# eezkni/UEGAN

Hardware: AMD Instinct MI355X
Metric: train imgs/sec @512px bs=16 on 1/2/4/8 MI355X; infer ms/img (higher is better)
Workload: dtype bf16; 1 GPU; FiveK-shaped 512x512 batch=16/GPU, full G/D/VGG train step (trainer.py:77-119), conv_dim=32, seeded stand-in VGG19; global_batch=16, parallelism=dp1, pool_size=50, collective=none (1 rank), passes=batched (fused.py)

## Files before the change

### uegan_amd/csrc/conv_wide.hip

```cpp
#include "conv_core.h"

namespace uegan {

static __device__ __attribute__((aligned(128))) const unsigned int g_zero_page[512] = {0u};

typedef float f32x16 __attribute__((ext_vector_type(16)));

__device__ __forceinline__ f32x16 mfma32_bf16(u32x4 a, u32x4 b, f32x16 c) {
#ifdef UEGAN_HALF_FP16
  return __builtin_amdgcn_mfma_f32_32x32x16_f16(__builtin_bit_cast(bf16x8_t, a), __builtin_bit_cast(bf16x8_t, b), c, 0, 0, 0);
#else
  return __builtin_amdgcn_mfma_f32_32x32x16_bf16(__builtin_bit_cast(bf16x8_t, a), __builtin_bit_cast(bf16x8_t, b), c, 0, 0, 0);
#endif
}

#define UEGAN_SB() __builtin_amdgcn_sched_barrier(0)

template <int KS, int MODE, bool MASK, int ABL = 0>
__global__ void __launch_bounds__(256, 1) conv_wide_kernel(ConvArgs a) {
  constexpr int TH = 8, TW = 32, BN = 256, NWAVES = 4;
  constexpr int PH = TH + KS - 1, PW = TW + KS - 1;
  constexpr int NPG = (PH * PW + 7) / 8;
  constexpr int NI_P = (NPG + NWAVES - 1) / NWAVES;
  constexpr int PBUFB = NPG * 1024, WHALF = BN * 64, DUMPB = 4096;
  constexpr int NT = KS * KS, NHC = 2 * NT;
  constexpr bool DGRAD = MODE != 0;
  static_assert(NI_P <= NHC - 2, "the next chunk's patch pieces must be requested two half steps before the chunk ends");
  static_assert(2 * PBUFB + 4 * WHALF + DUMPB + BN * 4 <= 160 * 1024, "LDS budget");

  __shared__ __attribute__((aligned(16))) unsigned char lds[2 * PBUFB + 4 * WHALF + DUMPB + BN * 4];
  unsigned char* const lds_w = lds + 2 * PBUFB;
  unsigned char* const lds_dump = lds_w + 4 * WHALF;
  unsigned char* const lds_bias = lds_dump + DUMPB;

  const ConvGeom& g = a.g;
  const bf16_t* in1 = static_cast<const bf16_t*>(a.in1);
  const bf16_t* w = static_cast<const bf16_t*>(a.w);
  const int tid = threadIdx.x, lane = tid & 63;
  const int wave = __builtin_amdgcn_readfirstlane(tid >> 6);
  const int wn = wave & 1, wm = wave >> 1;
  const int l31 = lane & 31, lh = lane >> 5;
  int n0 = blockIdx.y * BN;
  int t = blockIdx.x;
  if (a.xcd_map) {
    const int L = blockIdx.x + gridDim.x * blockIdx.y, nby = gridDim.y;
    const int xcd = L & 7, grp = L >> 3;
    n0 = (grp % nby) * BN;
    t = (grp / nby) * 8 + xcd;
  }
  const int tile_x = t % a.ntx; t /= a.ntx;
  const int tile_y = t % a.nty;
  const int b = t / a.nty;
  const int y0 = a.rect_y0 + tile_y * TH, x0 = a.rect_x0 + tile_x * TW;
  const int nchunk = g.C / 64;
  const int nsteps = nchunk * NT, nhs = 2 * nsteps;

  const int srow = lane >> 3, spos = lane & 7;
  const int c_in_chunk = (spos ^ (((lane >> 4) + 4 * (wave & 1)) & 7)) * 8;
  const unsigned char* pptr[NI_P];
  {
    const int vy0 = DGRAD ? y0 + g.pad - (KS - 1) : y0 - g.pad;
    const int vx0 = DGRAD ? x0 + g.pad - (KS - 1) : x0 - g.pad;
    const bool refl = !DGRAD && g.pad_mode == UEGAN_PAD_REFLECT;
#pragma unroll
    for (int ii = 0; ii < NI_P; ++ii) {
      const int pr = (ii * NWAVES + wave) * 8 + srow;
      const unsigned char* ptr = reinterpret_cast<const unsigned char*>(g_zero_page);
      if (pr < PH * PW) {
        const int piy = pr / PW, pix = pr - piy * PW;
        int sy = vy0 + piy, sx = vx0 + pix;
        if (refl) { sy = reflect_idx(sy, g.IH); sx = reflect_idx(sx, g.IW); }
        if (sy >= 0 && sy < g.IH && sx >= 0 && sx < g.IW)
          ptr = reinterpret_cast<const unsigned char*>(in1 + ((size_t)(b * g.IH + sy) * g.IW + sx) * g.C1 + c_in_chunk);
      }
      pptr[ii] = ptr;
    }
  }
  const unsigned char* p_src = pptr[0];
  unsigned char* p_dst = lds_dump;
  auto patch_piece_prepare = [&](int ii, int chunk, bool live) {
    const int rg = ii * NWAVES + wave;
    live = live && rg < NPG;
    p_src = pptr[ii < NI_P ? ii : 0] + (live ? chunk * 128 : 0);
    p_dst = live ? lds + (chunk & 1) * PBUFB + rg * 1024 : lds_dump + wave * 1024;
  };
  auto patch_piece_issue = [&]() { if (!(ABL & 1)) glds16(p_src, p_dst); };
  const bf16_t* const wlane = w + (size_t)(n0 + wave * 16 + (lane >> 2)) * a.Kp + (((lane & 3) ^ ((lane >> 4) & 3)) << 3);
  const size_t wrow64 = (size_t)64 * a.Kp;
  int s_chunk = 0, s_tap = 0, s_half = 0, s_hs = 0;
  const bf16_t* wsrc_cur = wlane;
  unsigned char* wdst_cur = lds_w;
  int wdst_stride = 4096;
  auto stage_w_prepare = [&]() {
    const bool live = s_hs < nhs;
    wsrc_cur = wlane + (s_tap * g.C + s_chunk * 64 + s_half * 32);
    wdst_cur = live ? lds_w + (s_hs & 3) * WHALF + wave * 1024 : lds_dump + wave * 1024;
    wdst_stride = live ? 4096 : 0;
    ++s_hs;
    s_half ^= 1;
    s_tap += s_half == 0 ? 1 : 0;
    const int wrap = s_tap == NT ? 1 : 0;
    s_tap = wrap ? 0 : s_tap;
    s_chunk = (s_chunk + wrap < nchunk) ? s_chunk + wrap : nchunk - 1;
  };
  auto stage_w_piece = [&](int i) { if (!(ABL & 1) || s_hs <= 3) glds16(wsrc_cur + (size_t)i * wrow64, wdst_cur + i * wdst_stride); };

  int wad[4];
#pragma unroll
  for (int i = 0; i < 4; ++i) wad[i] = (wn * 128 + i * 32 + l31) * 64 + ((lh ^ ((l31 >> 2) & 3)) << 4);
  int xad[4];
  auto set_xad1 = [&](int tap, int j) {
    const int ty = tap / KS, tx = tap - ty * KS;
    const int pty = DGRAD ? KS - 1 - ty : ty, ptx = DGRAD ? KS - 1 - tx : tx;
    const int pr = (wm * 4 + j + pty) * PW + l31 + ptx;
    xad[j] = pr * 128 + ((lh ^ ((pr >> 1) & 7)) << 4);
  };
  u32x4 wf0[4], xf0[4], wf1[4], xf1[4];
  f32x16 acc[4][4];
#pragma unroll
  for (int i = 0; i < 4; ++i)
#pragma unroll
    for (int j = 0; j < 4; ++j)
#pragma unroll
      for (int r = 0; r < 16; ++r) acc[i][j][r] = 0.f;

  const bool plain = !a.scale && !a.bias && a.act == UEGAN_ACT_NONE;
  if (!(ABL & 1)) {
    const int n = n0 + wave * 64 + lane;
    const bool live = !plain && a.bias && n < a.nbias;
    __builtin_amdgcn_global_load_lds((const __attribute__((address_space(1))) void*)(live ? a.bias + n : reinterpret_cast<const float*>(g_zero_page) + lane),
                                     (__attribute__((address_space(3))) void*)(lds_bias + wave * 256), 4, 0, 0);
  }
#pragma unroll
  for (int ii = 0; ii < NI_P; ++ii) { patch_piece_prepare(ii, 0, true); patch_piece_issue(); }
#pragma unroll
  for (int h = 0; h < 3; ++h) {
    stage_w_prepare();
#pragma unroll
    for (int i = 0; i < 4; ++i) stage_w_piece(i);
  }
  wait_vmcnt<4>();
  raw_barrier();
#pragma unroll
  for (int j = 0; j < 4; ++j) set_xad1(0, j);
#pragma unroll
  for (int i = 0; i < 4; ++i) wf0[i] = *reinterpret_cast<const u32x4*>(lds_w + wad[i]);
#pragma unroll
  for (int j = 0; j < 4; ++j) xf0[j] = *reinterpret_cast<const u32x4*>(lds + xad[j]);

#define MF(W, X, i, j) acc[i][j] = mfma32_bf16(W[i], X[j], acc[i][j]); UEGAN_SB();
#define LDW(F, slot, ksub, i) if (!(ABL & 2)) F[i] = *reinterpret_cast<const u32x4*>((slot) + (wad[i] ^ ((ksub) << 5)));
#define LDX(F, pb, kq, j) if (!(ABL & 2)) F[j] = *reinterpret_cast<const u32x4*>((pb) + (xad[j] ^ ((kq) << 5)));
  int chunk = 0, tap = 0;
  for (int step = 0; step < nsteps; ++step) {
    const unsigned char* pcur = lds + (chunk & 1) * PBUFB;
    const unsigned char* ws0 = lds_w + (step & 1) * (2 * WHALF);
    const unsigned char* ws1 = ws0 + WHALF;
    UEGAN_SB();
    MF(wf0, xf0, 0, 0) stage_w_prepare(); UEGAN_SB();
    MF(wf0, xf0, 0, 1) stage_w_piece(0); UEGAN_SB();
    MF(wf0, xf0, 0, 2) stage_w_piece(1); UEGAN_SB();
    MF(wf0, xf0, 0, 3) stage_w_piece(2); UEGAN_SB();
    MF(wf0, xf0, 1, 0) stage_w_piece(3); UEGAN_SB();
    MF(wf0, xf0, 1, 1) patch_piece_prepare(2 * tap, chunk + 1, 2 * tap < NI_P && chunk + 1 < nchunk); UEGAN_SB();
    MF(wf0, xf0, 1, 2) patch_piece_issue(); UEGAN_SB();
    MF(wf0, xf0, 1, 3) LDW(wf1, ws0, 1, 0) LDW(wf1, ws0, 1, 1) UEGAN_SB();
    MF(wf0, xf0, 2, 0) LDW(wf1, ws0, 1, 2) LDW(wf1, ws0, 1, 3) UEGAN_SB();
    MF(wf0, xf0, 2, 1) LDX(xf1, pcur, 1, 0) LDX(xf1, pcur, 1, 1) UEGAN_SB();
    MF(wf0, xf0, 2, 2) LDX(xf1, pcur, 1, 2) LDX(xf1, pcur, 1, 3) UEGAN_SB();
    MF(wf0, xf0, 2, 3) MF(wf0, xf0, 3, 0) MF(wf0, xf0, 3, 1) MF(wf0, xf0, 3, 2) MF(wf0, xf0, 3, 3)
    MF(wf1, xf1, 0, 0) MF(wf1, xf1, 0, 1) MF(wf1, xf1, 0, 2) MF(wf1, xf1, 0, 3)
    MF(wf1, xf1, 1, 0) LDW(wf0, ws1, 0, 0) LDW(wf0, ws1, 0, 1) UEGAN_SB();
    MF(wf1, xf1, 1, 1) LDW(wf0, ws1, 0, 2) LDW(wf0, ws1, 0, 3) UEGAN_SB();
    MF(wf1, xf1, 1, 2) LDX(xf0, pcur, 2, 0) LDX(xf0, pcur, 2, 1) UEGAN_SB();
    MF(wf1, xf1, 1, 3) LDX(xf0, pcur, 2, 2) LDX(xf0, pcur, 2, 3) UEGAN_SB();
    MF(wf1, xf1, 2, 0) MF(wf1, xf1, 2, 1) MF(wf1, xf1, 2, 2) MF(wf1, xf1, 2, 3)
    MF(wf1, xf1, 3, 0) MF(wf1, xf1, 3, 1) MF(wf1, xf1, 3, 2) MF(wf1, xf1, 3, 3)
    wait_vmcnt<5>();
    if (ABL < 4) raw_barrier();
    UEGAN_SB();
    MF(wf0, xf0, 0, 0) stage_w_prepare(); UEGAN_SB();
    MF(wf0, xf0, 0, 1) stage_w_piece(0); UEGAN_SB();
    MF(wf0, xf0, 0, 2) stage_w_piece(1); UEGAN_SB();
    MF(wf0, xf0, 0, 3) stage_w_piece(2); UEGAN_SB();
    MF(wf0, xf0, 1, 0) stage_w_piece(3); UEGAN_SB();
    MF(wf0, xf0, 1, 1) patch_piece_prepare(2 * tap + 1, chunk + 1, 2 * tap + 1 < NI_P && chunk + 1 < nchunk); UEGAN_SB();
    MF(wf0, xf0, 1, 2) patch_piece_issue(); UEGAN_SB();
    MF(wf0, xf0, 1, 3) LDW(wf1, ws1, 1, 0) LDW(wf1, ws1, 1, 1) UEGAN_SB();
    MF(wf0, xf0, 2, 0) LDW(wf1, ws1, 1, 2) LDW(wf1, ws1, 1, 3) UEGAN_SB();
    MF(wf0, xf0, 2, 1) LDX(xf1, pcur, 3, 0) LDX(xf1, pcur, 3, 1) UEGAN_SB();
    MF(wf0, xf0, 2, 2) LDX(xf1, pcur, 3, 2) LDX(xf1, pcur, 3, 3) UEGAN_SB();
    MF(wf0, xf0, 2, 3) MF(wf0, xf0, 3, 0) MF(wf0, xf0, 3, 1) MF(wf0, xf0, 3, 2) MF(wf0, xf0, 3, 3)
    {
      const int wrap = tap + 1 == NT ? 1 : 0;
      tap = wrap ? 0 : tap + 1;
      chunk += wrap;
    }
    const unsigned char* pnext = lds + (chunk & 1) * PBUFB;
    const unsigned char* wnext = lds_w + ((step + 1) & 1) * (2 * WHALF);
    MF(wf1, xf1, 0, 0) set_xad1(tap, 0); UEGAN_SB();
    MF(wf1, xf1, 0, 1) set_xad1(tap, 1); UEGAN_SB();
    MF(wf1, xf1, 0, 2) set_xad1(tap, 2); UEGAN_SB();
    MF(wf1, xf1, 0, 3) set_xad1(tap, 3); UEGAN_SB();
    MF(wf1, xf1, 1, 0) LDW(wf0, wnext, 0, 0) LDW(wf0, wnext, 0, 1) UEGAN_SB();
    MF(wf1, xf1, 1, 1) LDW(wf0, wnext, 0, 2) LDW(wf0, wnext, 0, 3) UEGAN_SB();
    MF(wf1, xf1, 1, 2) LDX(xf0, pnext, 0, 0) LDX(xf0, pnext, 0, 1) UEGAN_SB();
    MF(wf1, xf1, 1, 3) LDX(xf0, pnext, 0, 2) LDX(xf0, pnext, 0, 3) UEGAN_SB();
    MF(wf1, xf1, 2, 0) MF(wf1, xf1, 2, 1) MF(wf1, xf1, 2, 2) MF(wf1, xf1, 2, 3)
    MF(wf1, xf1, 3, 0) MF(wf1, xf1, 3, 1) MF(wf1, xf1, 3, 2) MF(wf1, xf1, 3, 3)
    wait_vmcnt<5>();
    if (ABL < 4) raw_barrier();
  }
#undef MF
#undef LDW
#undef LDX
  wait_vmcnt<0>();

  constexpr int EROW = 264;
  static_assert(4 * 128 * EROW <= 2 * PBUFB + 4 * WHALF, "epilogue staging fits the main loop's LDS");
  unsigned char* const est = lds + wave * (128 * EROW);
  {
    const float scale = a.scale ? a.scale[a.scale_group ? b / a.scale_group : 0] : 1.f;
    const float slope = a.act == UEGAN_ACT_LRELU ? 0.2f : (a.act == UEGAN_ACT_RELU ? 0.f : 1.f);
#pragma unroll
    for (int i = 0; i < 4; ++i) {
      f32x4 bv[4];
#pragma unroll
      for (int q = 0; q < 4; ++q) bv[q] = *reinterpret_cast<const f32x4*>(lds_bias + (wn * 128 + i * 32 + 4 * lh + 8 * q) * 4);
#pragma unroll
      for (int j = 0; j < 4; ++j) {
        unsigned char* row = est + (j * 32 + l31) * EROW + i * 64 + 8 * lh;
#pragma unroll
        for (int q = 0; q < 4; ++q) {
          float v[4];
#pragma unroll
          for (int r = 0; r < 4; ++r) {
            const float z = plain ? acc[i][j][4 * q + r] : acc[i][j][4 * q + r] * scale + bv[q][r];
            v[r] = plain ? z : fmaxf(z, slope * z);
          }
          u32x2 pk;
          pk.x = pack_bf16x2(v[0], v[1]);
          pk.y = pack_bf16x2(v[2], v[3]);
          *reinterpret_cast<u32x2*>(row + q * 16) = pk;
        }
      }
    }
  }
  __builtin_amdgcn_wave_barrier();
  {
    const float mslope = a.mask_act == UEGAN_ACT_LRELU ? 0.2f : (a.mask_act == UEGAN_ACT_RELU ? 0.f : 1.f);
    bf16_t* out = static_cast<bf16_t*>(a.out);
    const int nl = n0 + wn * 128 + (lane & 15) * 8;
#pragma unroll 4
    for (int it = 0; it < 32; ++it) {
      const int rr = it * 4 + (lane >> 4);
      const int oy = y0 + wm * 4 + (rr >> 5), ox = x0 + (rr & 31);
      const u32x2 v01 = *reinterpret_cast<const u32x2*>(est + rr * EROW + (lane & 15) * 16);
      const u32x2 v23 = *reinterpret_cast<const u32x2*>(est + rr * EROW + (lane & 15) * 16 + 8);
      u32x4 v = {v01.x, v01.y, v23.x, v23.y};
      if (oy >= g.OH || ox >= g.OW) continue;
      const size_t pix = ((size_t)b * g.OH + oy) * g.OW + ox;
      const size_t o = pix * a.N + nl;
      if (MASK) {
        const u32x4 m = *reinterpret_cast<const u32x4*>(static_cast<const bf16_t*>(a.mask) + o);
#pragma unroll
        for (int d = 0; d < 4; ++d) {
          const float lo = half_lo_to_f32(v[d]) * (half_lo_to_f32(m[d]) > 0.f ? 1.f : mslope);
          const float hi = half_hi_to_f32(v[d]) * (half_hi_to_f32(m[d]) > 0.f ? 1.f : mslope);
          v[d] = pack_bf16x2(lo, hi);
        }
      }
      bf16_t* dst = !a.out2 ? out + o : (nl < a.n_out1 ? out + pix * a.n_out1 + nl : static_cast<bf16_t*>(a.out2) + pix * (a.N - a.n_out1) + (nl - a.n_out1));
      *reinterpret_cast<u32x4*>(dst) = v;
    }
  }
}

template <int NI, int MODE, bool MASK, bool POOL, int RPW = 4, int EPI = 0>
__global__ void __launch_bounds__(256, RPW == 2 ? 2 : 1) conv_tall_kernel(ConvArgs a) {
  static_assert(RPW == 4 || RPW == 2, "rows per wave");
  constexpr bool REFL = MODE == 2;
  static_assert(!REFL || (NI == 4 && !MASK && !POOL), "mirrored images: 128-channel blocks, plain epilogue");
  static_assert(EPI == 0 || (MODE == 1 && MASK && !POOL), "fidelity-loss epilogues: masked data gradients");
  constexpr int KS = 3, TH = 4 * RPW, TW = 32, BN = NI * 32, NWAVES = 4;
  constexpr int PH = TH + KS - 1, PW = TW + KS - 1, NPIX = PH * PW;
  constexpr int NPG = (NPIX + 15) / 16;
  constexpr int NI_P = (NPG + NWAVES - 1) / NWAVES;
  constexpr int PBUFB = NPG * 1024, WSL = BN * 64, NWP = WSL / 1024 / NWAVES;
  constexpr int DUMPB = RPW == 2 ? 1024 : 4096, DUMPW = RPW == 2 ? 0 : 1024;
  constexpr int NT = KS * KS, NLOAD = NWP + 2;
  constexpr bool DGRAD = MODE != 0;
  constexpr int EROW = BN * 2 + 8;
  constexpr int WPIX = RPW * 32;
  constexpr int MAINB = 2 * PBUFB + 4 * WSL, EPIB = NWAVES * WPIX * EROW;
  constexpr int BODYB = MAINB > EPIB ? MAINB : EPIB;
  static_assert(NI_P <= 2 * (NT - 2), "the next chunk's patch pieces must be requested two steps before the chunk ends");
  static_assert((RPW == 2 ? 2 : 1) * (BODYB + DUMPB + BN * 4) <= 160 * 1024, "LDS budget");
  static_assert(NWP >= 1, "at least one weight piece per wave per slice");

  __shared__ __attribute__((aligned(16))) unsigned char lds[BODYB + DUMPB + BN * 4];
  unsigned char* const lds_w = lds + 2 * PBUFB;
  unsigned char* const lds_dump = lds + BODYB;
  unsigned char* const lds_bias = lds_dump + DUMPB;

  const ConvGeom& g = a.g;
  const bf16_t* in1 = static_cast<const bf16_t*>(a.in1);
  const bf16_t* in2 = static_cast<const bf16_t*>(a.in2);
  const bf16_t* w = static_cast<const bf16_t*>(a.w);
  const int tid = threadIdx.x, lane = tid & 63;
  const int wave = __builtin_amdgcn_readfirstlane(tid >> 6);
  const int l31 = lane & 31, lh = lane >> 5;
  int n0 = blockIdx.y * BN;
  int t = blockIdx.x;
  if (a.xcd_map) {
    const int L = blockIdx.x + gridDim.x * blockIdx.y, nby = gridDim.y;
    const int xcd = L & 7, grp = L >> 3;
    n0 = (grp % nby) * BN;
    t = (grp / nby) * 8 + xcd;
  }
  const int tile_x = t % a.ntx; t /= a.ntx;
  const int tile_y = t % a.nty;
  const int b = t / a.nty;
  const int y0 = a.rect_y0 + tile_y * TH, x0 = a.rect_x0 + tile_x * TW;
  const int nchunk = g.C / 32, nchunk1 = g.C1 / 32;
  const int nsteps = nchunk * NT;

  const int q_src = ((lane & 3) ^ ((lane >> 4) & 3)) * 8;
  int ppix[NI_P];
  {
    const int vy0 = DGRAD ? y0 + g.pad - (KS - 1) : y0 - g.pad;
    const int vx0 = DGRAD ? x0 + g.pad - (KS - 1) : x0 - g.pad;
    const bool refl = !DGRAD && g.pad_mode == UEGAN_PAD_REFLECT;
#pragma unroll
    for (int ii = 0; ii < NI_P; ++ii) {
      const int pr = (ii * NWAVES + wave) * 16 + (lane >> 2);
      int pix = -1;
      if (pr < NPIX) {
        const int piy = pr / PW, pix_x = pr - piy * PW;
        int sy = vy0 + piy, sx = vx0 + pix_x;
        if (refl) { sy = reflect_idx(sy, g.IH); sx = reflect_idx(sx, g.IW); }
        if (sy >= 0 && sy < g.IH && sx >= 0 && sx < g.IW) pix = (b * g.IH + sy) * g.IW + sx;
      }
      ppix[ii] = pix;
    }
  }
  const unsigned char* const zero16 = reinterpret_cast<const unsigned char*>(g_zero_page) + (lane & 3) * 16;
  const unsigned char* p_src = zero16;
  unsigned char* p_dst = lds_dump;
  auto patch_piece_prepare = [&](int pidx, int chunk, bool live) {
    const int rg = pidx * NWAVES + wave;
    live = live && pidx < NI_P && rg < NPG;
    const int pix = ppix[pidx < NI_P ? pidx : 0];
    const bool first = chunk < nchunk1;
    const bf16_t* base = first ? in1 : in2;
    const int cs = first ? g.C1 : g.C2, c0 = (first ? chunk : chunk - nchunk1) * 32 + q_src;
    p_src = (live && pix >= 0) ? reinterpret_cast<const unsigned char*>(base + ((size_t)pix * cs + c0)) : zero16;
    p_dst = live ? lds + (chunk & 1) * PBUFB + rg * 1024 : lds_dump + wave * DUMPW;
  };
  auto patch_piece_issue = [&]() { glds16(p_src, p_dst); };
  const bf16_t* const wlane = w + (size_t)(n0 + wave * 16 + (lane >> 2)) * a.Kp + q_src;
  const size_t wrow64 = (size_t)64 * a.Kp;
  int s_chunk = 0, s_tap = 0, s_idx = 0;
  const bf16_t* wsrc_cur = wlane;
  unsigned char* wdst_cur = lds_w;
  int wdst_stride = 4096;
  auto stage_w_prepare = [&]() {
    const bool live = s_idx < nsteps;
    wsrc_cur = wlane + (s_tap * g.C + s_chunk * 32);
    wdst_cur = live ? lds_w + (s_idx & 3) * WSL + wave * 1024 : lds_dump + wave * DUMPW;
    wdst_stride = live ? 4096 : 0;
    ++s_idx;
    ++s_tap;
    const int wrap = s_tap == NT ? 1 : 0;
    s_tap = wrap ? 0 : s_tap;
    s_chunk = (s_chunk + wrap < nchunk) ? s_chunk + wrap : nchunk - 1;
  };
  auto stage_w_piece = [&](int i) { glds16(wsrc_cur + (size_t)i * wrow64, wdst_cur + i * wdst_stride); };

  int wad[NI];
#pragma unroll
  for (int i = 0; i < NI; ++i) wad[i] = (i * 32 + l31) * 64 + ((lh ^ ((l31 >> 2) & 3)) << 4);
  const int xbase = wave * RPW * PW + l31;
  int xad[RPW];
  int xpr[REFL ? RPW : 1];
  auto set_xad = [&](int tap, int j) {
    const int ty = tap / KS, tx = tap - ty * KS;
    const int pty = DGRAD ? KS - 1 - ty : ty, ptx = DGRAD ? KS - 1 - tx : tx;
    const int pr = xbase + (j + pty) * PW + ptx;
    xad[j] = pr * 64 + ((lh ^ ((pr >> 2) & 3)) << 4);
    if constexpr (REFL) xpr[j] = pr;
  };
  bool r_top[RPW], r_bot[RPW];
  bool e_left = false, e_right = false, c_left = false, c_right = false, edge = false;
  if constexpr (REFL) {
#pragma unroll
    for (int j = 0; j < RPW; ++j) {
      const int y = y0 + wave * RPW + j;
      r_top[j] = y == 1;
      r_bot[j] = y == g.OH - 2;
      edge = edge || r_top[j] || r_bot[j];
    }
    e_left = x0 == 0;
    e_right = x0 <= g.OW - 2 && g.OW - 2 < x0 + TW;
    c_left = x0 + l31 == 1;
    c_right = x0 + l31 == g.OW - 2;
    edge = edge || e_left || e_right;
  } else {
#pragma unroll
    for (int j = 0; j < RPW; ++j) r_top[j] = r_bot[j] = false;
  }
  auto fold1 = [&](u32x4& F, const unsigned char* pb, int ksub, int j, int tap) {
    const int ty = tap / KS, tx = tap - ty * KS;
    const bool ym = ty == 0 ? r_top[j] : (ty == 2 ? r_bot[j] : false);
    const bool xany = tx == 0 ? e_left : (tx == 2 ? e_right : false);
    if (!ym && !xany) return;
    const int dpy = ty == 0 ? -2 * PW : 2 * PW, dpx = tx == 0 ? -2 : 2;
    auto rd = [&](int pr) { return *reinterpret_cast<const u32x4*>(pb + ((pr * 64 + ((lh ^ ((pr >> 2) & 3)) << 4)) ^ (ksub << 5))); };
    if (ym) F = add_frag<bf16_t>(F, rd(xpr[j] + dpy));
    if (xany) {
      const uint32_t m = (tx == 0 ? c_left : c_right) ? 0xffffffffu : 0u;
      u32x4 v = rd(xpr[j] + dpx);
      if (ym) v = add_frag<bf16_t>(v, rd(xpr[j] + dpy + dpx));
      F = add_frag<bf16_t>(F, v & u32x4{m, m, m, m});
    }
  };
  u32x4 wf0[NI], xf0[RPW], wf1[NI], xf1[RPW];
  f32x16 acc[NI][RPW];
#pragma unroll
  for (int i = 0; i < NI; ++i)
#pragma unroll
    for (int j = 0; j < RPW; ++j)
#pragma unroll
      for (int r = 0; r < 16; ++r) acc[i][j][r] = 0.f;
  const bool plain = !a.scale && !a.bias && a.act == UEGAN_ACT_NONE;
  {
    const int n = n0 + wave * 64 + lane;
    const bool live = wave * 64 < BN && !plain && a.bias && n < a.nbias;
    __builtin_amdgcn_global_load_lds((const __attribute__((address_space(1))) void*)(live ? a.bias + n : reinterpret_cast<const float*>(g_zero_page) + lane),
                                     (__attribute__((address_space(3))) void*)(wave * 64 < BN ? lds_bias + wave * 256 : lds_dump + wave * DUMPW), 4, 0, 0);
  }
  const float scale = a.scale ? a.scale[a.scale_group ? b / a.scale_group : 0] : 1.f;

#pragma unroll
  for (int ii = 0; ii < NI_P; ++ii) { patch_piece_prepare(ii, 0, true); patch_piece_issue(); }
#pragma unroll
  for (int h = 0; h < 3; ++h) {
    stage_w_prepare();
#pragma unroll
    for (int i = 0; i < NWP; ++i) stage_w_piece(i);
  }
  wait_vmcnt<NWP>();
  raw_barrier();
#pragma unroll
  for (int j = 0; j < RPW; ++j) set_xad(0, j);
#pragma unroll
  for (int i = 0; i < NI; ++i) wf0[i] = *reinterpret_cast<const u32x4*>(lds_w + wad[i]);
#pragma unroll
  for (int j = 0; j < RPW; ++j) xf0[j] = *reinterpret_cast<const u32x4*>(lds + xad[j]);

#define MF(W, X, i, j) acc[i][j] = mfma32_bf16(W[i], X[j], acc[i][j]); UEGAN_SB();
#define LDW(F, slot, ksub, i) F[i] = *reinterpret_cast<const u32x4*>((slot) + (wad[i] ^ ((ksub) << 5)));
#define LDX(F, pb, ksub, j) F[j] = *reinterpret_cast<const u32x4*>((pb) + (xad[j] ^ ((ksub) << 5)));
#define FOLDX(F, pb, ksub, tapv)                                                           \
  if constexpr (REFL) {                                                                    \
    if (edge) {                                                                            \
      _Pragma("unroll") for (int jf = 0; jf < RPW; ++jf) fold1(F[jf], pb, ksub, jf, tapv); \
    }                                                                                      \
  }
  FOLDX(xf0, lds, 0, 0)
  for (int chunk = 0; chunk < nchunk; ++chunk) {
    const unsigned char* pcur = lds + (chunk & 1) * PBUFB;
    const bool more = chunk + 1 < nchunk;
#pragma unroll
    for (int tap = 0; tap < NT; ++tap) {
      const int step = chunk * NT + tap;
      const unsigned char* ws = lds_w + (step & 3) * WSL;
      const unsigned char* wnext = lds_w + ((step + 1) & 3) * WSL;
      const unsigned char* pnext = tap + 1 == NT ? lds + ((chunk + 1) & 1) * PBUFB : pcur;
      const int ntap = tap + 1 == NT ? 0 : tap + 1;
      UEGAN_SB();
      if constexpr (RPW == 2 && NI == 2) {
        MF(wf0, xf0, 0, 0) LDW(wf1, ws, 1, 0) LDW(wf1, ws, 1, 1) UEGAN_SB();
        MF(wf0, xf0, 0, 1) LDX(xf1, pcur, 1, 0) LDX(xf1, pcur, 1, 1) UEGAN_SB();
        MF(wf0, xf0, 1, 0) stage_w_prepare(); stage_w_piece(0); UEGAN_SB();
        if (2 * tap < NI_P) {
          MF(wf0, xf0, 1, 1) patch_piece_prepare(2 * tap, chunk + 1, more); patch_piece_issue(); patch_piece_prepare(2 * tap + 1, chunk + 1, more); patch_piece_issue(); UEGAN_SB();
        } else {
          MF(wf0, xf0, 1, 1)
        }
        MF(wf1, xf1, 0, 0) set_xad(ntap, 0); set_xad(ntap, 1); UEGAN_SB();
        MF(wf1, xf1, 0, 1) LDW(wf0, wnext, 0, 0) LDW(wf0, wnext, 0, 1) UEGAN_SB();
        MF(wf1, xf1, 1, 0) LDX(xf0, pnext, 0, 0) LDX(xf0, pnext, 0, 1) UEGAN_SB();
        MF(wf1, xf1, 1, 1)
      } else if constexpr (RPW == 2) {
        MF(wf0, xf0, 0, 0) LDW(wf1, ws, 1, 0) LDW(wf1, ws, 1, 1) UEGAN_SB();
        MF(wf0, xf0, 0, 1) LDW(wf1, ws, 1, 2) LDW(wf1, ws, 1, 3) UEGAN_SB();
        MF(wf0, xf0, 1, 0) LDX(xf1, pcur, 1, 0) LDX(xf1, pcur, 1, 1) UEGAN_SB();
        MF(wf0, xf0, 1, 1) stage_w_prepare(); UEGAN_SB();
        MF(wf0, xf0, 2, 0) stage_w_piece(0); UEGAN_SB();
        MF(wf0, xf0, 2, 1) stage_w_piece(1); UEGAN_SB();
        MF(wf0, xf0, 3, 0) patch_piece_prepare(2 * tap, chunk + 1, more); UEGAN_SB();
        MF(wf0, xf0, 3, 1) patch_piece_issue(); patch_piece_prepare(2 * tap + 1, chunk + 1, more); patch_piece_issue(); UEGAN_SB();
        FOLDX(xf1, pcur, 1, tap)
        MF(wf1, xf1, 0, 0) set_xad(ntap, 0); set_xad(ntap, 1); UEGAN_SB();
        MF(wf1, xf1, 0, 1) LDW(wf0, wnext, 0, 0) LDW(wf0, wnext, 0, 1) UEGAN_SB();
        MF(wf1, xf1, 1, 0) LDW(wf0, wnext, 0, 2) LDW(wf0, wnext, 0, 3) UEGAN_SB();
        MF(wf1, xf1, 1, 1) LDX(xf0, pnext, 0, 0) LDX(xf0, pnext, 0, 1) UEGAN_SB();
        MF(wf1, xf1, 2, 0) MF(wf1, xf1, 2, 1) MF(wf1, xf1, 3, 0) MF(wf1, xf1, 3, 1)
        FOLDX(xf0, pnext, 0, ntap)
      } else if constexpr (NI == 4) {
        MF(wf0, xf0, 0, 0) stage_w_prepare(); UEGAN_SB();
        MF(wf0, xf0, 0, 1) stage_w_piece(0); UEGAN_SB();
        MF(wf0, xf0, 0, 2) stage_w_piece(1); UEGAN_SB();
        MF(wf0, xf0, 0, 3) patch_piece_prepare(2 * tap, chunk + 1, more); UEGAN_SB();
        MF(wf0, xf0, 1, 0) patch_piece_issue(); UEGAN_SB();
        MF(wf0, xf0, 1, 1) patch_piece_prepare(2 * tap + 1, chunk + 1, more); UEGAN_SB();
        MF(wf0, xf0, 1, 2) patch_piece_issue(); UEGAN_SB();
        MF(wf0, xf0, 1, 3) LDW(wf1, ws, 1, 0) LDW(wf1, ws, 1, 1) UEGAN_SB();
        MF(wf0, xf0, 2, 0) LDW(wf1, ws, 1, 2) LDW(wf1, ws, 1, 3) UEGAN_SB();
        MF(wf0, xf0, 2, 1) LDX(xf1, pcur, 1, 0) LDX(xf1, pcur, 1, 1) UEGAN_SB();
        MF(wf0, xf0, 2, 2) LDX(xf1, pcur, 1, 2) LDX(xf1, pcur, 1, 3) UEGAN_SB();
        MF(wf0, xf0, 2, 3) MF(wf0, xf0, 3, 0) MF(wf0, xf0, 3, 1) MF(wf0, xf0, 3, 2) MF(wf0, xf0, 3, 3)
        FOLDX(xf1, pcur, 1, tap)
        MF(wf1, xf1, 0, 0) set_xad(ntap, 0); UEGAN_SB();
        MF(wf1, xf1, 0, 1) set_xad(ntap, 1); UEGAN_SB();
        MF(wf1, xf1, 0, 2) set_xad(ntap, 2); UEGAN_SB();
        MF(wf1, xf1, 0, 3) set_xad(ntap, 3); UEGAN_SB();
        MF(wf1, xf1, 1, 0) LDW(wf0, wnext, 0, 0) LDW(wf0, wnext, 0, 1) UEGAN_SB();
        MF(wf1, xf1, 1, 1) LDW(wf0, wnext, 0, 2) LDW(wf0, wnext, 0, 3) UEGAN_SB();
        MF(wf1, xf1, 1, 2) LDX(xf0, pnext, 0, 0) LDX(xf0, pnext, 0, 1) UEGAN_SB();
        MF(wf1, xf1, 1, 3) LDX(xf0, pnext, 0, 2) LDX(xf0, pnext, 0, 3) UEGAN_SB();
        MF(wf1, xf1, 2, 0) MF(wf1, xf1, 2, 1) MF(wf1, xf1, 2, 2) MF(wf1, xf1, 2, 3)
        MF(wf1, xf1, 3, 0) MF(wf1, xf1, 3, 1) MF(wf1, xf1, 3, 2) MF(wf1, xf1, 3, 3)
        FOLDX(xf0, pnext, 0, ntap)
      } else {
        static_assert(NI == 2 || NI == 4, "channel fragments per wave");
        MF(wf0, xf0, 0, 0) LDW(wf1, ws, 1, 0) LDW(wf1, ws, 1, 1) UEGAN_SB();
        MF(wf0, xf0, 0, 1) LDX(xf1, pcur, 1, 0) LDX(xf1, pcur, 1, 1) UEGAN_SB();
        MF(wf0, xf0, 0, 2) LDX(xf1, pcur, 1, 2) LDX(xf1, pcur, 1, 3) UEGAN_SB();
        MF(wf0, xf0, 0, 3) stage_w_prepare(); UEGAN_SB();
        MF(wf0, xf0, 1, 0) stage_w_piece(0); UEGAN_SB();
        MF(wf0, xf0, 1, 1) patch_piece_prepare(2 * tap, chunk + 1, more); UEGAN_SB();
        MF(wf0, xf0, 1, 2) patch_piece_issue(); patch_piece_prepare(2 * tap + 1, chunk + 1, more); UEGAN_SB();
        MF(wf0, xf0, 1, 3) patch_piece_issue(); UEGAN_SB();
        MF(wf1, xf1, 0, 0) set_xad(ntap, 0); set_xad(ntap, 1); UEGAN_SB();
        MF(wf1, xf1, 0, 1) set_xad(ntap, 2); set_xad(ntap, 3); LDW(wf0, wnext, 0, 0) LDW(wf0, wnext, 0, 1) UEGAN_SB();
        MF(wf1, xf1, 0, 2) LDX(xf0, pnext, 0, 0) LDX(xf0, pnext, 0, 1) UEGAN_SB();
        MF(wf1, xf1, 0, 3) LDX(xf0, pnext, 0, 2) LDX(xf0, pnext, 0, 3) UEGAN_SB();
        MF(wf1, xf1, 1, 0) MF(wf1, xf1, 1, 1) MF(wf1, xf1, 1, 2) MF(wf1, xf1, 1, 3)
      }
      if (RPW == 2 && NI == 2 && 2 * tap >= NI_P) wait_vmcnt<NWP>();
      else wait_vmcnt<NLOAD>();
      raw_barrier();
    }
  }
#undef MF
#undef LDW
#undef LDX
#undef FOLDX
  wait_vmcnt<0>();

  unsigned char* const est = lds + wave * (WPIX * EROW);
  float tst[EPI == 1 ? 32 : 1], ttot[EPI == 1 ? 24 : 1], tgs = 1.f;
  if constexpr (EPI == 1) {
    const size_t bc = (size_t)g.B * a.N, o0 = (size_t)b * a.N + n0 + (lane % (BN / 8)) * 8;
#pragma unroll
    for (int q = 0; q < 8; ++q) {
      const f32x4 v = *reinterpret_cast<const f32x4*>(a.epi_st + (q >> 1) * bc + o0 + 4 * (q & 1));
#pragma unroll
      for (int e = 0; e < 4; ++e) tst[4 * q + e] = v[e];
    }
#pragma unroll
    for (int q = 0; q < 6; ++q) {
      const f32x4 v = *reinterpret_cast<const f32x4*>(a.epi_tot + o0 * 3 + 4 * q);
#pragma unroll
      for (int e = 0; e < 4; ++e) ttot[4 * q + e] = v[e];
    }
    if (a.epi_gscale) tgs = *a.epi_gscale;
  }
  {
    const float slope = a.act == UEGAN_ACT_LRELU ? 0.2f : (a.act == UEGAN_ACT_RELU ? 0.f : 1.f);
#pragma unroll
    for (int i = 0; i < NI; ++i) {
      f32x4 bv[4];
#pragma unroll
      for (int q = 0; q < 4; ++q) bv[q] = *reinterpret_cast<const f32x4*>(lds_bias + (i * 32 + 4 * lh + 8 * q) * 4);
#pragma unroll
      for (int j = 0; j < RPW; ++j) {
        unsigned char* row = est + (j * 32 + l31) * EROW + i * 64 + 8 * lh;
#pragma unroll
        for (int q = 0; q < 4; ++q) {
          float v[4];
#pragma unroll
          for (int r = 0; r < 4; ++r) {
            const float z = plain ? acc[i][j][4 * q + r] : acc[i][j][4 * q + r] * scale + bv[q][r];
            v[r] = plain ? z : fmaxf(z, slope * z);
          }
          u32x2 pk;
          pk.x = pack_bf16x2(v[0], v[1]);
          pk.y = pack_bf16x2(v[2], v[3]);
          *reinterpret_cast<u32x2*>(row + q * 16) = pk;
        }
      }
    }
  }
  __builtin_amdgcn_wave_barrier();
  {
    constexpr int LPP = BN / 8;
    constexpr int PPI = 64 / LPP;
    const float mslope = a.mask_act == UEGAN_ACT_LRELU ? 0.2f : (a.mask_act == UEGAN_ACT_RELU ? 0.f : 1.f);
    bf16_t* out = static_cast<bf16_t*>(a.out);
    const int lc = lane % LPP, nl = n0 + lc * 8;
    const int n_store = (POOL && b >= a.n_full) ? 0 : WPIX / PPI;
    float tmx[EPI == 1 ? 8 : 1], trx[EPI == 1 ? 8 : 1], tmy[EPI == 1 ? 8 : 1], try_[EPI == 1 ? 8 : 1], tmg[EPI == 1 ? 8 : 1], tmgx[EPI == 1 ? 8 : 1];
    float tk = 0.f;
    if constexpr (EPI == 1) {
      float inv_n;
      percep_scalars(a.epi_weight, &tgs, g.B, g.OH * g.OW, a.N, tk, inv_n);
#pragma unroll
      for (int e = 0; e < 8; ++e) percep_consts(tst, ttot, 8, e, tk, inv_n, tmx[e], trx[e], tmy[e], try_[e], tmg[e], tmgx[e]);
    }
#pragma unroll 4
    for (int it = 0; it < n_store; ++it) {
      const int rr = it * PPI + lane / LPP;
      const int oy = y0 + wave * RPW + (rr >> 5), ox = x0 + (rr & 31);
      const u32x2 v01 = *reinterpret_cast<const u32x2*>(est + rr * EROW + lc * 16);
      const u32x2 v23 = *reinterpret_cast<const u32x2*>(est + rr * EROW + lc * 16 + 8);
      u32x4 v = {v01.x, v01.y, v23.x, v23.y};
      if (oy >= g.OH || ox >= g.OW) continue;
      const size_t pix = ((size_t)b * g.OH + oy) * g.OW + ox;
      const size_t o = pix * a.N + nl;
      if (MASK) {
        const u32x4 m = *reinterpret_cast<const u32x4*>(static_cast<const bf16_t*>(a.mask) + o);
        u32x4 yv = {0u, 0u, 0u, 0u};
        if constexpr (EPI == 1) yv = *reinterpret_cast<const u32x4*>(static_cast<const bf16_t*>(a.epi_y) + o);
#pragma unroll
        for (int d = 0; d < 4; ++d) {
          float lo = half_lo_to_f32(v[d]) * (half_lo_to_f32(m[d]) > 0.f ? 1.f : mslope);
          float hi = half_hi_to_f32(v[d]) * (half_hi_to_f32(m[d]) > 0.f ? 1.f : mslope);
          if constexpr (EPI == 1) {
            const float xl = half_lo_to_f32(m[d]), xh = half_hi_to_f32(m[d]);
            const float gl = percep_tap_grad(xl, half_lo_to_f32(yv[d]), tmx[2 * d], trx[2 * d], tmy[2 * d], try_[2 * d], tk, tmg[2 * d], tmgx[2 * d]);
            const float gh = percep_tap_grad(xh, half_hi_to_f32(yv[d]), tmx[2 * d + 1], trx[2 * d + 1], tmy[2 * d + 1], try_[2 * d + 1], tk,
                                             tmg[2 * d + 1], tmgx[2 * d + 1]);
            lo = (xl > 0.f ? gl : 0.f) + lo;
            hi = (xh > 0.f ? gh : 0.f) + hi;
          }
          v[d] = pack_bf16x2(lo, hi);
        }
      }
      if constexpr (EPI == 2) {
        const u32x2 a8 = *reinterpret_cast<const u32x2*>(a.epi_idx + o);
        const size_t ow2 = 2 * (size_t)g.OW;
        bf16_t* base = out + (((size_t)b * 2 * g.OH + 2 * oy) * ow2 + 2 * ox) * a.N + nl;
#pragma unroll
        for (int k = 0; k < 4; ++k) {
          u32x4 w4;
#pragma unroll
          for (int d = 0; d < 4; ++d) {
            const uint32_t by = a8[d >> 1] >> (16 * (d & 1));
            w4[d] = v[d] & (((by & 0xffu) == (uint32_t)k ? 0xffffu : 0u) | (((by >> 8) & 0xffu) == (uint32_t)k ? 0xffff0000u : 0u));
          }
          *reinterpret_cast<u32x4*>(base + ((k >> 1) * ow2 + (k & 1)) * a.N) = w4;
        }
        continue;
      }
      bf16_t* dst = !a.out2 ? out + o : (nl < a.n_out1 ? out + pix * a.n_out1 + nl : static_cast<bf16_t*>(a.out2) + pix * (a.N - a.n_out1) + (nl - a.n_out1));
      *reinterpret_cast<u32x4*>(dst) = v;
    }
    if constexpr (POOL) {
      bf16_t* pout = static_cast<bf16_t*>(a.pool_out);
      const int PH2 = g.OH >> 1, PW2 = g.OW >> 1;
#pragma unroll 2
      for (int it = 0; it < WPIX / 4 / PPI; ++it) {
        const int pp = it * PPI + lane / LPP;
        const int pr = pp >> 4, pc = pp & 15;
        const int py = ((y0 + wave * RPW) >> 1) + pr, px = (x0 >> 1) + pc;
        float m[8];
        uint32_t arg[8];
#pragma unroll
        for (int e = 0; e < 8; ++e) { m[e] = -3.0e38f; arg[e] = 0; }
#pragma unroll
        for (int dy = 0; dy < 2; ++dy)
#pragma unroll
          for (int dx = 0; dx < 2; ++dx) {
            const int rr = (2 * pr + dy) * 32 + 2 * pc + dx;
            const u32x2 v01 = *reinterpret_cast<const u32x2*>(est + rr * EROW + lc * 16);
            const u32x2 v23 = *reinterpret_cast<const u32x2*>(est + rr * EROW + lc * 16 + 8);
            const uint32_t vv[4] = {v01.x, v01.y, v23.x, v23.y};
#pragma unroll
            for (int d = 0; d < 4; ++d) {
              const float lo = half_lo_to_f32(vv[d]), hi = half_hi_to_f32(vv[d]);
              if (lo > m[2 * d]) { m[2 * d] = lo; arg[2 * d] = dy * 2 + dx; }
              if (hi > m[2 * d + 1]) { m[2 * d + 1] = hi; arg[2 * d + 1] = dy * 2 + dx; }
            }
          }
        if (py >= PH2 || px >= PW2) continue;
        const size_t po = (((size_t)b * PH2 + py) * PW2 + px) * a.N + nl;
        u32x4 o4 = {pack_bf16x2(m[0], m[1]), pack_bf16x2(m[2], m[3]), pack_bf16x2(m[4], m[5]), pack_bf16x2(m[6], m[7])};
        *reinterpret_cast<u32x4*>(pout + po) = o4;
        if (a.pool_idx && b < a.n_idx) {
          const u32x2 a8 = {arg[0] | (arg[1] << 8) | (arg[2] << 16) | (arg[3] << 24), arg[4] | (arg[5] << 8) | (arg[6] << 16) | (arg[7] << 24)};
          *reinterpret_cast<u32x2*>(static_cast<unsigned char*>(a.pool_idx) + po) = a8;
        }
      }
    }
  }
}

int conv_tall_run(ConvArgs& a, int dtype, hipStream_t s, bool interior) {
  const ConvGeom& g = a.g;
  const int min_grid = g_tuning[UEGAN_TUNE_TALL_MIN_GRID];
  if (min_grid < 0) return 1;
  if (dtype != UEGAN_BF16 || g.stride != 1 || g.KH != 3 || g.KW != 3 || a.frame != 0) return 1;
  if (g.C1 % 32 || g.C2 % 32 || g.C > 1024 || (a.N != 64 && a.N % 128) || g.OW < 32 || g.OH < 16) return 1;
  const bool refl = !interior && g.mode == 1 && g.pad_mode == UEGAN_PAD_REFLECT && g.pad == 1 && !g.C2 && !a.mask && a.N % 128 == 0 &&
                    (!a.out2 || a.n_out1 % 8 == 0) && g.OH >= 4 && g.OW >= 4 && g_tuning[UEGAN_TUNE_TALL_REFLECT] != 0;
  if (!interior && !refl && (a.out2 || (g.mode == 1 && (g.C2 || (g.pad_mode == UEGAN_PAD_REFLECT && g.pad != 0))))) return 1;
  if (interior && (g.mode != 1 || g.C2 || a.mask || (a.out2 && a.n_out1 % 8))) return 1;
  auto simple = [](int act) { return act == UEGAN_ACT_NONE || act == UEGAN_ACT_LRELU || act == UEGAN_ACT_RELU; };
  if (!simple(a.act) || (a.mask && !simple(a.mask_act))) return 1;
  if (a.epi && (interior || refl || g.mode != 1 || !a.mask || a.mask_act != UEGAN_ACT_RELU || a.out2 || g.C2)) return 1;
  const int rpw_knob = g_tuning[UEGAN_TUNE_TALL_RPW];
  bool rpw2 = rpw_knob == 2 || (rpw_knob != 4 && g.C < 512);
  const int nb_n = a.N == 64 ? 1 : a.N / 128;
  {
    const int ntx = interior ? (a.rect_x1 - a.rect_x0) / 32 : (g.OW + 31) / 32;
    const int nty16 = interior ? (a.rect_y1 - a.rect_y0) / 16 : (g.OH + 15) / 16, nty8 = interior ? (a.rect_y1 - a.rect_y0) / 8 : (g.OH + 7) / 8;
    if (g.B * nty16 * ntx * nb_n < min_grid) {
      if (rpw_knob == 4 || g.B * nty8 * ntx * nb_n < min_grid) return 1;
      rpw2 = true;
    }
  }
  const int th = rpw2 ? 8 : 16;
  a.nty = interior ? (a.rect_y1 - a.rect_y0) / th : (g.OH + th - 1) / th;
  a.ntx = interior ? (a.rect_x1 - a.rect_x0) / 32 : (g.OW + 31) / 32;
  const int gm = g.B * a.nty * a.ntx;
  const bool pool = a.pool_out && g.mode == 0 && !a.mask && g.OH % 2 == 0 && g.OW % 2 == 0;
  const double rows = interior ? (double)g.B * (a.rect_y1 - a.rect_y0) * (a.rect_x1 - a.rect_x0) : (g.mode == 0 ? (double)g.B * g.OH * g.OW : (double)g.B * g.IH * g.IW);
  ProfScope prof(prof_key(7, true, a.N == 64 ? 64 : 128, 3, refl ? 2 : g.mode, 16, !pool), 2.0 * rows * a.N * (double)(9 * g.C), s,
                 2.0 * (rows * a.N + (interior ? rows : (double)g.B * g.IH * g.IW) * g.C));
  const dim3 grid(gm, a.N == 64 ? 1 : a.N / 128), block(256);
  a.xcd_map = (grid.y > 1 && gm % 8 == 0) ? 1 : 0;
#define UEGAN_TALL(NI, RPW)                                                                                          \
  do {                                                                                                               \
    if (g.mode == 0 && pool) hipLaunchKernelGGL((conv_tall_kernel<NI, 0, false, true, RPW>), grid, block, 0, s, a);  \
    else if (g.mode == 0) hipLaunchKernelGGL((conv_tall_kernel<NI, 0, false, false, RPW>), grid, block, 0, s, a);    \
    else if (a.mask && a.epi == 1) hipLaunchKernelGGL((conv_tall_kernel<NI, 1, true, false, RPW, 1>), grid, block, 0, s, a); \
    else if (a.mask && a.epi == 2) hipLaunchKernelGGL((conv_tall_kernel<NI, 1, true, false, RPW, 2>), grid, block, 0, s, a); \
    else if (a.mask) hipLaunchKernelGGL((conv_tall_kernel<NI, 1, true, false, RPW>), grid, block, 0, s, a);          \
    else hipLaunchKernelGGL((conv_tall_kernel<NI, 1, false, false, RPW>), grid, block, 0, s, a);                     \
  } while (0)
  if (refl) {
    if (rpw2) hipLaunchKernelGGL((conv_tall_kernel<4, 2, false, false, 2>), grid, block, 0, s, a);
    else hipLaunchKernelGGL((conv_tall_kernel<4, 2, false, false, 4>), grid, block, 0, s, a);
  }
  else if (a.N == 64) { if (rpw2) UEGAN_TALL(2, 2); else UEGAN_TALL(2, 4); }
  else if (rpw2) UEGAN_TALL(4, 2);
  else UEGAN_TALL(4, 4);
#undef UEGAN_TALL
  if (g.mode == 0 && pool) a.pool_done = 1;
  UEGAN_CHECK_LAUNCH();
  return UEGAN_OK;
}

int conv_wide_run(ConvArgs& a, int dtype, hipStream_t s, bool interior) {
  const ConvGeom& g = a.g;
  const int min_grid = g_tuning[UEGAN_TUNE_WIDE_MIN_GRID];
  if (min_grid < 0) return 1;
  if (dtype != UEGAN_BF16 || g.stride != 1 || g.KH != 3 || g.KW != 3 || a.frame != 0) return 1;
  if (g.C % 64 || g.C > 1024 || g.C2 || a.N % 256 || g.OW < 32 || g.OH < 8) return 1;
  if (!interior && (a.out2 || (g.mode == 1 && g.pad_mode == UEGAN_PAD_REFLECT && g.pad != 0))) return 1;
  if (interior && (g.mode != 1 || a.mask || (a.out2 && a.n_out1 % 8))) return 1;
  auto simple = [](int act) { return act == UEGAN_ACT_NONE || act == UEGAN_ACT_LRELU || act == UEGAN_ACT_RELU; };
  if (!simple(a.act) || (a.mask && !simple(a.mask_act))) return 1;
  a.nty = interior ? (a.rect_y1 - a.rect_y0) / 8 : (g.OH + 7) / 8;
  a.ntx = interior ? (a.rect_x1 - a.rect_x0) / 32 : (g.OW + 31) / 32;
  const int gm = g.B * a.nty * a.ntx;
  if (gm * (a.N / 256) < min_grid) return 1;
  const double rows = interior ? (double)g.B * (a.rect_y1 - a.rect_y0) * (a.rect_x1 - a.rect_x0) : (g.mode == 0 ? (double)g.B * g.OH * g.OW : (double)g.B * g.IH * g.IW);
  ProfScope prof(prof_key(7, true, 256, 3, g.mode, 8, true), 2.0 * rows * a.N * (double)(9 * g.C), s,
                 2.0 * (rows * a.N + (interior ? rows : (double)g.B * g.IH * g.IW) * g.C));
  const dim3 grid(gm, a.N / 256), block(256);
  const int nby = a.N / 256;
  a.xcd_map = (nby > 1 && gm % 8 == 0) ? 1 : 0;
#ifdef UEGAN_TOOLS_BUILD
  const int abl = g_abl_wide;
  if (g.mode == 0 && abl == 1) hipLaunchKernelGGL((conv_wide_kernel<3, 0, false, 1>), grid, block, 0, s, a);
  else if (g.mode == 0 && abl == 2) hipLaunchKernelGGL((conv_wide_kernel<3, 0, false, 2>), grid, block, 0, s, a);
  else if (g.mode == 0 && abl == 3) hipLaunchKernelGGL((conv_wide_kernel<3, 0, false, 3>), grid, block, 0, s, a);
  else if (g.mode == 0 && abl == 4) hipLaunchKernelGGL((conv_wide_kernel<3, 0, false, 7>), grid, block, 0, s, a);
  else
#endif
  if (g.mode == 0) hipLaunchKernelGGL((conv_wide_kernel<3, 0, false>), grid, block, 0, s, a);
  else if (a.mask) hipLaunchKernelGGL((conv_wide_kernel<3, 1, true>), grid, block, 0, s, a);
  else hipLaunchKernelGGL((conv_wide_kernel<3, 1, false>), grid, block, 0, s, a);
  UEGAN_CHECK_LAUNCH();
  return UEGAN_OK;
}

int conv_interior_run(ConvArgs& a, int dtype, hipStream_t s) {
  const ConvGeom& g = a.g;
  if (dtype != UEGAN_BF16 || g.mode != 1 || g.stride != 1 || g.KH != 3 || g.KW != 3 || g.pad_mode != UEGAN_PAD_REFLECT || g.pad != 1 || a.frame != 0 || a.mask)
    return 1;
  const int y0 = 16, y1 = (g.OH - 1 - g.pad) / 16 * 16, x0 = 16, x1 = 16 + (g.OW - 1 - g.pad - 16) / 32 * 32;
  if (y1 <= y0 || x1 <= x0 || 2LL * (y1 - y0) * (x1 - x0) < (long long)g.OH * g.OW) return 1;
  a.rect_y0 = y0; a.rect_y1 = y1; a.rect_x0 = x0; a.rect_x1 = x1;
  int rc = conv_tall_run(a, dtype, s, true);
  if (rc == 1) rc = conv_wide_run(a, dtype, s, true);
  if (rc != UEGAN_OK) { a.rect_y0 = a.rect_y1 = a.rect_x0 = a.rect_x1 = 0; return rc; }
  a.border_only = 1;
  return UEGAN_OK;
}

}
```

Baseline: 499.4 imgs/sec.

## Batch and prefetch mask loads in masked conv epilogues, double-buffered

```diff
diff --git a/uegan_amd/csrc/conv_wide.hip b/uegan_amd/csrc/conv_wide.hip
--- a/uegan_amd/csrc/conv_wide.hip
+++ b/uegan_amd/csrc/conv_wide.hip
@@ -15,6 +15,17 @@
 }
 
 #define UEGAN_SB() __builtin_amdgcn_sched_barrier(0)
+
+constexpr int EPI_NB = 8;
+template <int EPI>
+struct EpiBatch {
+  u32x4 m[EPI_NB];
+  u32x4 y[EPI == 1 ? EPI_NB : 1];
+  u32x2 idx[EPI == 2 ? EPI_NB : 1];
+};
+constexpr int tall_epi_fetch_at(int ni, int rpw, int epi) {
+  return ni == 4 && epi == 1 ? 2 : (ni == 4 && rpw == 4 ? ni : 0);
+}
 
 template <int KS, int MODE, bool MASK, int ABL = 0>
 __global__ void __launch_bounds__(256, 1) conv_wide_kernel(ConvArgs a) {
@@ -219,6 +230,24 @@
   constexpr int EROW = 264;
   static_assert(4 * 128 * EROW <= 2 * PBUFB + 4 * WHALF, "epilogue staging fits the main loop's LDS");
   unsigned char* const est = lds + wave * (128 * EROW);
+  constexpr int NB = EPI_NB, NBATCH = 32 / NB;
+  static_assert(NBATCH % 2 == 0, "batches in pairs");
+  EpiBatch<0> eb0, eb1;
+  auto epi_pixel = [&](int it, int& rr, int& oy, int& ox) {
+    rr = it * 4 + (lane >> 4);
+    oy = y0 + wm * 4 + (rr >> 5);
+    ox = x0 + (rr & 31);
+    return oy < g.OH && ox < g.OW;
+  };
+  auto epi_fetch = [&](int bt, EpiBatch<0>& q) {
+#pragma unroll
+    for (int k = 0; k < NB; ++k) {
+      int rr, oy, ox;
+      const bool ok = epi_pixel(bt * NB + k, rr, oy, ox);
+      const size_t o = (((size_t)b * g.OH + (ok ? oy : y0)) * g.OW + (ok ? ox : x0)) * a.N + n0 + wn * 128 + (lane & 15) * 8;
+      q.m[k] = *reinterpret_cast<const u32x4*>(static_cast<const bf16_t*>(a.mask) + o);
+    }
+  };
   {
     const float scale = a.scale ? a.scale[a.scale_group ? b / a.scale_group : 0] : 1.f;
     const float slope = a.act == UEGAN_ACT_LRELU ? 0.2f : (a.act == UEGAN_ACT_RELU ? 0.f : 1.f);
@@ -247,12 +276,13 @@
     }
   }
   __builtin_amdgcn_wave_barrier();
+  if constexpr (MASK) epi_fetch(0, eb0);
   {
     const float mslope = a.mask_act == UEGAN_ACT_LRELU ? 0.2f : (a.mask_act == UEGAN_ACT_RELU ? 0.f : 1.f);
     bf16_t* out = static_cast<bf16_t*>(a.out);
     const int nl = n0 + wn * 128 + (lane & 15) * 8;
 #pragma unroll 4
-    for (int it = 0; it < 32; ++it) {
+    for (int it = 0; it < (MASK ? 0 : 32); ++it) {
       const int rr = it * 4 + (lane >> 4);
       const int oy = y0 + wm * 4 + (rr >> 5), ox = x0 + (rr & 31);
       const u32x2 v01 = *reinterpret_cast<const u32x2*>(est + rr * EROW + (lane & 15) * 16);
@@ -261,17 +291,35 @@
       if (oy >= g.OH || ox >= g.OW) continue;
       const size_t pix = ((size_t)b * g.OH + oy) * g.OW + ox;
       const size_t o = pix * a.N + nl;
-      if (MASK) {
-        const u32x4 m = *reinterpret_cast<const u32x4*>(static_cast<const bf16_t*>(a.mask) + o);
+      bf16_t* dst = !a.out2 ? out + o : (nl < a.n_out1 ? out + pix * a.n_out1 + nl : static_cast<bf16_t*>(a.out2) + pix * (a.N - a.n_out1) + (nl - a.n_out1));
+      *reinterpret_cast<u32x4*>(dst) = v;
+    }
+    auto epi_store = [&](int bt, const EpiBatch<0>& q) {
+#pragma unroll
+      for (int k = 0; k < NB; ++k) {
+        int rr, oy, ox;
+        const bool ok = epi_pixel(bt * NB + k, rr, oy, ox);
+        const u32x2 v01 = *reinterpret_cast<const u32x2*>(est + rr * EROW + (lane & 15) * 16);
+        const u32x2 v23 = *reinterpret_cast<const u32x2*>(est + rr * EROW + (lane & 15) * 16 + 8);
+        u32x4 v = {v01.x, v01.y, v23.x, v23.y};
+        const u32x4 m = q.m[k];
 #pragma unroll
         for (int d = 0; d < 4; ++d) {
           const float lo = half_lo_to_f32(v[d]) * (half_lo_to_f32(m[d]) > 0.f ? 1.f : mslope);
           const float hi = half_hi_to_f32(v[d]) * (half_hi_to_f32(m[d]) > 0.f ? 1.f : mslope);
           v[d] = pack_bf16x2(lo, hi);
         }
-      }
-      bf16_t* dst = !a.out2 ? out + o : (nl < a.n_out1 ? out + pix * a.n_out1 + nl : static_cast<bf16_t*>(a.out2) + pix * (a.N - a.n_out1) + (nl - a.n_out1));
-      *reinterpret_cast<u32x4*>(dst) = v;
+        if (ok) *reinterpret_cast<u32x4*>(out + (((size_t)b * g.OH + oy) * g.OW + ox) * a.N + nl) = v;
+      }
+    };
+    if constexpr (MASK) {
+#pragma unroll 1
+      for (int bt = 0; bt < NBATCH; bt += 2) {
+        epi_fetch(bt + 1, eb1);
+        epi_store(bt, eb0);
+        if (bt + 2 < NBATCH) epi_fetch(bt + 2, eb0);
+        epi_store(bt + 1, eb1);
+      }
     }
   }
 }
@@ -578,10 +626,38 @@
     }
     if (a.epi_gscale) tgs = *a.epi_gscale;
   }
+  constexpr int LPP = BN / 8;
+  constexpr int PPI = 64 / LPP;
+  constexpr int NS = WPIX / PPI;
+  const int lcm = MASK ? lane % LPP : 0, nlm = n0 + lcm * 8;
+  constexpr int NB = EPI_NB, NBATCH = NS / NB;
+  static_assert(NS % NB == 0 && (NBATCH <= 2 || NBATCH % 2 == 0), "whole batches, in pairs");
+  EpiBatch<EPI> eb0, eb1;
+  auto epi_pixel = [&](int it, int& rr, int& oy, int& ox) {
+    rr = it * PPI + lane / LPP;
+    oy = y0 + wave * RPW + (rr >> 5);
+    ox = x0 + (rr & 31);
+    return oy < g.OH && ox < g.OW;
+  };
+  auto epi_fetch = [&](int bt, EpiBatch<EPI>& q) {
+#pragma unroll
+    for (int k = 0; k < NB; ++k) {
+      int rr, oy, ox;
+      const bool ok = epi_pixel(bt * NB + k, rr, oy, ox);
+      const size_t o = (((size_t)b * g.OH + (ok ? oy : y0)) * g.OW + (ok ? ox : x0)) * a.N + nlm;
+      q.m[k] = *reinterpret_cast<const u32x4*>(static_cast<const bf16_t*>(a.mask) + o);
+      if constexpr (EPI == 1) q.y[k] = *reinterpret_cast<const u32x4*>(static_cast<const bf16_t*>(a.epi_y) + o);
+      if constexpr (EPI == 2) q.idx[k] = *reinterpret_cast<const u32x2*>(a.epi_idx + o);
+    }
+  };
+  constexpr int EFA = tall_epi_fetch_at(NI, RPW, EPI);
   {
     const float slope = a.act == UEGAN_ACT_LRELU ? 0.2f : (a.act == UEGAN_ACT_RELU ? 0.f : 1.f);
 #pragma unroll
     for (int i = 0; i < NI; ++i) {
+      if constexpr (MASK) {
+        if (i == EFA) { epi_fetch(0, eb0); UEGAN_SB(); }
+      }
       f32x4 bv[4];
 #pragma unroll
       for (int q = 0; q < 4; ++q) bv[q] = *reinterpret_cast<const f32x4*>(lds_bias + (i * 32 + 4 * lh + 8 * q) * 4);
@@ -605,13 +681,12 @@
     }
   }
   __builtin_amdgcn_wave_barrier();
+  if constexpr (MASK && EFA == NI) { epi_fetch(0, eb0); UEGAN_SB(); }
   {
-    constexpr int LPP = BN / 8;
-    constexpr int PPI = 64 / LPP;
     const float mslope = a.mask_act == UEGAN_ACT_LRELU ? 0.2f : (a.mask_act == UEGAN_ACT_RELU ? 0.f : 1.f);
     bf16_t* out = static_cast<bf16_t*>(a.out);
     const int lc = lane % LPP, nl = n0 + lc * 8;
-    const int n_store = (POOL && b >= a.n_full) ? 0 : WPIX / PPI;
+    const int n_store = (MASK || (POOL && b >= a.n_full)) ? 0 : NS;
     float tmx[EPI == 1 ? 8 : 1], trx[EPI == 1 ? 8 : 1], tmy[EPI == 1 ? 8 : 1], try_[EPI == 1 ? 8 : 1], tmg[EPI == 1 ? 8 : 1], tmgx[EPI == 1 ? 8 : 1];
     float tk = 0.f;
     if constexpr (EPI == 1) {
@@ -630,15 +705,24 @@
       if (oy >= g.OH || ox >= g.OW) continue;
       const size_t pix = ((size_t)b * g.OH + oy) * g.OW + ox;
       const size_t o = pix * a.N + nl;
-      if (MASK) {
-        const u32x4 m = *reinterpret_cast<const u32x4*>(static_cast<const bf16_t*>(a.mask) + o);
-        u32x4 yv = {0u, 0u, 0u, 0u};
-        if constexpr (EPI == 1) yv = *reinterpret_cast<const u32x4*>(static_cast<const bf16_t*>(a.epi_y) + o);
+      bf16_t* dst = !a.out2 ? out + o : (nl < a.n_out1 ? out + pix * a.n_out1 + nl : static_cast<bf16_t*>(a.out2) + pix * (a.N - a.n_out1) + (nl - a.n_out1));
+      *reinterpret_cast<u32x4*>(dst) = v;
+    }
+    auto epi_store = [&](int bt, const EpiBatch<EPI>& q) {
+#pragma unroll
+      for (int k = 0; k < NB; ++k) {
+        int rr, oy, ox;
+        const bool ok = epi_pixel(bt * NB + k, rr, oy, ox);
+        const u32x2 v01 = *reinterpret_cast<const u32x2*>(est + rr * EROW + lcm * 16);
+        const u32x2 v23 = *reinterpret_cast<const u32x2*>(est + rr * EROW + lcm * 16 + 8);
+        u32x4 v = {v01.x, v01.y, v23.x, v23.y};
+        const u32x4 m = q.m[k];
 #pragma unroll
         for (int d = 0; d < 4; ++d) {
           float lo = half_lo_to_f32(v[d]) * (half_lo_to_f32(m[d]) > 0.f ? 1.f : mslope);
           float hi = half_hi_to_f32(v[d]) * (half_hi_to_f32(m[d]) > 0.f ? 1.f : mslope);
           if constexpr (EPI == 1) {
+            const u32x4 yv = q.y[k];
             const float xl = half_lo_to_f32(m[d]), xh = half_hi_to_f32(m[d]);
             const float gl = percep_tap_grad(xl, half_lo_to_f32(yv[d]), tmx[2 * d], trx[2 * d], tmy[2 * d], try_[2 * d], tk, tmg[2 * d], tmgx[2 * d]);
             const float gh = percep_tap_grad(xh, half_hi_to_f32(yv[d]), tmx[2 * d + 1], trx[2 * d + 1], tmy[2 * d + 1], try_[2 * d + 1], tk,
@@ -648,25 +732,39 @@
           }
           v[d] = pack_bf16x2(lo, hi);
         }
-      }
-      if constexpr (EPI == 2) {
-        const u32x2 a8 = *reinterpret_cast<const u32x2*>(a.epi_idx + o);
-        const size_t ow2 = 2 * (size_t)g.OW;
-        bf16_t* base = out + (((size_t)b * 2 * g.OH + 2 * oy) * ow2 + 2 * ox) * a.N + nl;
-#pragma unroll
-        for (int k = 0; k < 4; ++k) {
-          u32x4 w4;
-#pragma unroll
-          for (int d = 0; d < 4; ++d) {
-            const uint32_t by = a8[d >> 1] >> (16 * (d & 1));
-            w4[d] = v[d] & (((by & 0xffu) == (uint32_t)k ? 0xffffu : 0u) | (((by >> 8) & 0xffu) == (uint32_t)k ? 0xffff0000u : 0u));
+        if (!ok) continue;
+        if constexpr (EPI == 2) {
+          const u32x2 a8 = q.idx[k];
+          const size_t ow2 = 2 * (size_t)g.OW;
+          bf16_t* base = out + (((size_t)b * 2 * g.OH + 2 * oy) * ow2 + 2 * ox) * a.N + nlm;
+#pragma unroll
+          for (int kk = 0; kk < 4; ++kk) {
+            u32x4 w4;
+#pragma unroll
+            for (int d = 0; d < 4; ++d) {
+              const uint32_t by = a8[d >> 1] >> (16 * (d & 1));
+              w4[d] = v[d] & (((by & 0xffu) == (uint32_t)kk ? 0xffffu : 0u) | (((by >> 8) & 0xffu) == (uint32_t)kk ? 0xffff0000u : 0u));
+            }
+            *reinterpret_cast<u32x4*>(base + ((kk >> 1) * ow2 + (kk & 1)) * a.N) = w4;
           }
-          *reinterpret_cast<u32x4*>(base + ((k >> 1) * ow2 + (k & 1)) * a.N) = w4;
+        } else {
+          const size_t o = (((size_t)b * g.OH + oy) * g.OW + ox) * a.N + nlm;
+          *reinterpret_cast<u32x4*>(out + o) = v;
         }
-        continue;
-      }
-      bf16_t* dst = !a.out2 ? out + o : (nl < a.n_out1 ? out + pix * a.n_out1 + nl : static_cast<bf16_t*>(a.out2) + pix * (a.N - a.n_out1) + (nl - a.n_out1));
-      *reinterpret_cast<u32x4*>(dst) = v;
+      }
+    };
+    if constexpr (MASK && NBATCH <= 2) {
+      if constexpr (NBATCH == 2) { UEGAN_SB(); epi_fetch(1, eb1); }
+      epi_store(0, eb0);
+      if constexpr (NBATCH == 2) epi_store(1, eb1);
+    } else if constexpr (MASK) {
+#pragma unroll 1
+      for (int bt = 0; bt < NBATCH; bt += 2) {
+        epi_fetch(bt + 1, eb1);
+        epi_store(bt, eb0);
+        if (bt + 2 < NBATCH) epi_fetch(bt + 2, eb0);
+        epi_store(bt + 1, eb1);
+      }
     }
     if constexpr (POOL) {
       bf16_t* pout = static_cast<bf16_t*>(a.pool_out);
```

Result: no change. 500.2 imgs/sec, median of 6 (+0.2%).
